# kursawe/OpticalFlow

Hardware: AMD Instinct MI355X
Metric: frame-pairs/sec (higher is better)
Workload: dtype f64; 1 GPU; 1024x1024x256 synthetic translating texture (seed 1), speed_alpha=1, remodelling_alpha=1e4, rtol=1e-06, all 255 pairs solved to the stopping rule; frames_per_gpu=256, pairs_in_flight=255, levels=9, coarse_stencils=float8, vcycle_vectors=coarse_float32, w_cycle_level=1, w_cycle_visits=3, warm_start_stride=3, allgather=False, gather_chunks=1, converged=True

## Files before the change

opticalflow_amd/csrc/vof.hip:

```cpp
#include "vof_device.hpp"
#include "vof_sweep0r.hpp"
#include "vof_sweep0p.hpp"
#include "vof_stream0.hpp"
#include "vof_direct.hpp"
#include "vof_boxflow.hpp"
#include "vof_boxsweep.hpp"
#include "vof_blursweep.hpp"
#include "vof_compare.hpp"
#include "vof_liushen.hpp"
#include "../../include/vof.h"

#include <fcntl.h>
#include <unistd.h>

#include <algorithm>
#include <atomic>
#include <chrono>
#include <cmath>
#include <condition_variable>
#include <cstdio>
#include <cstdlib>
#include <cstring>
#include <mutex>
#include <string>
// ... 49 lines not shown
    size_t warm_cap = 0;
    int* warm_src = nullptr;
    double* partials = nullptr;
    int nblk = 0;
    PairScalars* sc = nullptr;
    int* active = nullptr;
    int* alist = nullptr;
    int alist_n = 0;
    bool use_alist = true;
    double* func3 = nullptr;
    double *W = nullptr, *invT = nullptr;
    int nd = 0;
    int* h_active = nullptr;
    int* h_alist = nullptr;
    PairScalars* h_sc = nullptr;
    double* h_func3 = nullptr;
    char* h_bounce = nullptr;
    hipEvent_t ev_batch[2] = {nullptr, nullptr};
    double* st_movie = nullptr;
    double* st_out[4] = {nullptr, nullptr, nullptr, nullptr};
    double* st_out2[4] = {nullptr, nullptr, nullptr, nullptr};
    hipStream_t copy_stream = nullptr;
    hipEvent_t ev_solved[2] = {nullptr, nullptr}, ev_copied[2] = {nullptr, nullptr}, ev_uploaded[2] = {nullptr, nullptr};
    double* st_movie2 = nullptr;
    double *blur_tmp = nullptr, *blur_w = nullptr, *blur_io = nullptr;
    double* bf_scratch = nullptr;
    double* sw_scratch = nullptr;
    size_t sw_planes = 0;
    bool sw_by_budget = false;
    char* sw_aux = nullptr;
    size_t sw_aux_bytes = 0;
    bool bf_lds_set = false;
    bool bl_lds_set = false;
    bool ls_lds_set = false;
    double* tex_tab = nullptr;
    size_t tex_cap = 0;
    double* gm_V = nullptr;
    GmresState* gm_state = nullptr;
    double* gm_partials = nullptr;
    int* gm_cycle = nullptr;
    int gm_m = 0;
    long long gmres_pairs = 0;
    struct Alloc { void* raw; char* user; size_t bytes; const char* name; int line; };
    std::vector<Alloc> allocs;
    int c_bytes_per_point = 0;
    size_t bytes = 0;
    std::string err;
    const double* frames = nullptr;
    int npairs = 0;
    vof_params prm;
    int cfmt = 0;
    bool fused = true;
    bool fold_stored = false;
    bool direct_on = false;
    int dir_cap = 0;
    double *dir_T = nullptr, *dir_tabs = nullptr, *dir_W = nullptr, *dir_r = nullptr, *dir_y = nullptr, *dir_x = nullptr, *dir_t = nullptr;
    int *dir_ipiv = nullptr, *dir_info = nullptr;
    double *dir_R = nullptr, *dir_C = nullptr, *dir_D = nullptr;
    int dir_ld = 0;
    long long direct_pairs = 0;
    bool fuse_rr = true;
    bool fuse_b = true;
    int fused_ends = 3;
    long sweep0r_min_blocks = 512;
    int tail_first = -1;
    size_t tail_lds = 0;
    TailArgs tail;
    int tail_key[6] = {-9, -9, -9, -9, -9, -9};
    bool prof = false;
    int prof_kid = -1, prof_level = -1;
    std::vector<ProfRec> recs;
    std::vector<hipEvent_t> free_events;
    long long prof_dropped = 0;
    double prof_ms[VOF_K_COUNT][16];
    long long prof_n[VOF_K_COUNT][16];
    long long prof_units[VOF_K_COUNT][16];
    double prof_bytes[VOF_K_COUNT][16];
    double prof_moved[VOF_K_COUNT][16];
    int cur_units = 0;
    int dbg_sync = 0;
    long long dbg_seq = 0;
    std::string dbg_fault;
    int dbg_fd = -1;
    bool dbg_canary = false;
    bool dbg_alloc_log = false;
    bool dbg_poison = false;
    size_t part_per_pair = 0;
    vof_ctx* lane_parent = nullptr;
    int lane_lo = 0, lane_slots = 0;
    int dir_ok = -1;
    hipStream_t lane_stream[MAX_LANES] = {};
    hipEvent_t lane_ev[MAX_LANES][2] = {};
    hipEvent_t ev_fork = nullptr;
    hipEvent_t group_ev[MAX_LANES * MAX_LANE_GROUPS] = {};
};

static std::string g_create_error;

namespace {

void dbg_sync_check(vof_ctx* c, const char* what, int level) {
    if (!c->dbg_sync) return;
    ++c->dbg_seq;
    char line[256];
    if (c->dbg_fd >= 0) {
        int n = snprintf(line, sizeof line, "in flight: scope #%lld '%s' level %d, %d pairs, grid %dx%d (%d levels)%-40s\n", c->dbg_seq, what, level,
// ... 356 lines not shown
}

template <typename VT, typename CVT = VT>
void resrestrict_fine_t(vof_ctx* c, const VT* x, const VT* b, CVT* bc, int np, ActiveSet active) {
    Level &f = c->L[0], &k = c->L[1];
    int TI = pick_band_height(f.ni, (k.nj + RR_CO - 1) / RR_CO, c->cur_units);
    dim3 g((k.nj + RR_CO - 1) / RR_CO, (k.ni + TI / 2 - 1) / (TI / 2), pair_slots(c, active, np));
    Prof p(c, VOF_K_APPLY0, 0, (8.0 + 6.0 * sizeof(VT)) * f.npts + 3.0 * sizeof(CVT) * k.npts);
    k_stream_resrestrict0<VT, VT, CVT><<<g, AP_THREADS, 0, c->stream>>>(ap_args(c, TI, active), x, b, bc, k.ni, k.nj);
}

inline double resu_coef_bytes(const vof_ctx* c) {
    return c->cfmt == 3 ? 12.0 * 4 : (c->cfmt == 2 ? 18.5 * 4 : (c->cfmt == 1 ? 36.0 * 4 : 36.0 * 8));
}
template <typename VT>
void resrestrict_u_t(vof_ctx* c, int l, const VT* x_new, const VT* x_old, VT* bc, int np, ActiveSet active) {
    Level &f = c->L[l], &k = c->L[l + 1];
    const double vs = sizeof(VT);
    const double algo = (coef_bytes(c, l) + 9.0 * vs) * f.npts + 3.0 * vs * (f.npts + k.npts);
    const double moved = (resu_coef_bytes(c) + (x_old ? 6.0 : 3.0) * vs) * f.npts + 3.0 * vs * k.npts;
    Prof p(c, VOF_K_RESIDUAL, l, algo, moved);
    dim3 g(1, (k.ni + BY - 1) / BY, pair_slots(c, active, np));
    CDISPATCH(c, l, {
        if (x_old) k_resrestrict_u<CT, VT, true><<<g, blk2d, 0, c->stream>>>((const CW*)f.C, f.ni, f.nj, x_new, x_old, bc, k.ni, k.nj, active);
        else k_resrestrict_u<CT, VT, false><<<g, blk2d, 0, c->stream>>>((const CW*)f.C, f.ni, f.nj, x_new, x_old, bc, k.ni, k.nj, active);
    });
}

template <typename VT>
void prolong_add_level_t(vof_ctx* c, int l, VT* fine, const VT* coarse, int np, ActiveSet active) {
    Level &f = c->L[l], &k = c->L[l + 1];
    Prof p(c, VOF_K_PROLONG, l, 3.0 * sizeof(VT) * (2 * f.npts + k.npts));
    k_prolong_add<VT><<<grid2d(f.ni, f.nj, pair_slots(c, active, np)), blk2d, 0, c->stream>>>(fine, f.ni, f.nj, coarse, k.ni, k.nj, active);
}

template <typename VT>
void coarse_solve_t(vof_ctx* c, const VT* r, VT* e, int np, ActiveSet active) {
    Prof p(c, VOF_K_COARSE_SOLVE, (int)c->L.size() - 1);
    k_coarse_solve<VT><<<pair_slots(c, active, np), 256, c->nd * sizeof(double), c->stream>>>(c->invT, c->nd, r, e, active);
}

inline bool sweep0m_usable(const vof_ctx* c) {
    return c->fused && !c->vfloat && (c->L[0].nj % 2 == 0) && c->L[0].C == nullptr;
}

inline bool sweep0p_usable(const vof_ctx* c) {
    return c->fused && c->vfloat && (c->L[0].nj % 2 == 0) && c->L[0].C == nullptr && c->prm.reference_quirks;
}

inline bool sweep_st_usable(const vof_ctx* c, int l) {
    return l > 0 && c->L[l].C != nullptr && c->cfmt >= 2;
}

inline bool coarse32_ok(const vof_ctx* c, int nu_post) {
    return c->vcoarse32 && c->L.size() > 1 && sweep0m_usable(c) && nu_post > 0;
}


struct CycleIO {
    S0Trail trail{nullptr, nullptr, 0, nullptr};
    S0BSrc bf{nullptr, nullptr, nullptr, nullptr, nullptr, nullptr};
    int bf_mode = 0;
    int trail_nblk = 0;
    bool rr_done = false;
    bool bf_done = false;
    bool failed = false;
};

struct L0Req {
    bool from_zero = false;
    int po = 0;
    int nsweeps = 1;
    bool ec = false, ec32 = false;
    bool trail = false, trail_dot = false;
    bool rr = false, rr_f32 = false;
    int bf = 0;
    bool x32 = false;
};

enum L0Family { L0_SWEEP0R, L0_SWEEP0M, L0_SWEEP0P, L0_SWEEP0 };

struct L0Pass {
    L0Family fam = L0_SWEEP0;
    int NS = 1;
    bool EC = false, FROM_ZERO = false;
    int TRAIL = 0;
    bool ET32 = false;
    int PO = 0;
    int BF = 0;
    bool XT32 = false;
    int nx = 0, nxp = 0, ny = 0, TI = 0, nci = 0, ncj = 0;
    unsigned blocks = 0, block = 0;
    size_t lds = 0;
    double algo = 0.0, moved = 0.0;
    bool trail() const { return TRAIL == 1; }
    bool rr() const { return TRAIL == 2; }
    int bf() const { return BF == 3 ? 0 : BF; }
};

struct S0Geo { int nx, ny, TI; bool s0r; };
inline S0Geo s0_geometry(const vof_ctx* c, int rows, int NSW, bool trail) {
    const Level& lv = c->L[0];
    S0Geo g;
    const int out = S0_W - 8 * NSW - (trail ? 4 : 0);
    g.nx = (lv.nj + out - 1) / out;
    g.TI = pick_band_height(rows, g.nx, c->cur_units);
// ... 241 lines not shown
        {
            Prof pr(c, VOF_K_GS0, 0, p.algo, p.moved);
            const int nslots = pair_slots(c, active, np);
            switch (p.fam) {
                case L0_SWEEP0R: launched = launch_s0r(c, p, f0, nslots, ptrs); break;
                case L0_SWEEP0M: launched = launch_s0m(c, p, f0, nslots, ptrs); break;
                case L0_SWEEP0P: launched = launch_s0p(c, p, f0, nslots, ptrs); break;
                case L0_SWEEP0: launched = launch_s0<VT>(c, p, f0, nslots, ptrs); break;
            }
        }
        if (!launched) { c->err = "internal: the library holds no kernel for the planned level-0 pass"; io.failed = true; return; }
        if (p.trail()) io.trail_nblk = (int)p.blocks;
        if (p.rr()) io.rr_done = true;
        if (p.bf()) { io.bf_done = true; if (p.bf() == 1) fold_s_epilogue(c, np, p); }
        return;
    }
    const int rows = lv.ni + po;
    const int W = GeoB::W;
    const int nx = (lv.nj + GeoB::OUT - 1) / GeoB::OUT;
    const int TI = pick_band_height(rows, nx, c->cur_units);
    const int ny = (rows + TI - 1) / TI;
    const int nslots = pair_slots(c, active, np);
    dim3 g((unsigned)nx * ny * nslots, 1, 1);
    const double vs = sizeof(VT);
    int nci = 0, ncj = 0;
    double ebytes = 0.0;
    if (ecoarse) { nci = c->L[l + 1].ni; ncj = c->L[l + 1].nj; ebytes = 3.0 * vs * c->L[l + 1].npts; }
    Prof p(c, VOF_K_GS, l, (coef_bytes(c, l) + (x_in ? 9.0 : 6.0) * vs) * lv.npts + ebytes);
    size_t lds = (size_t)(SW_RING * 3 * W) * sizeof(VT);
    if (sweep_st_usable(c, l)) {
        const uint32_t* Cw = (const uint32_t*)lv.C;
        auto launch = [&](auto ct_tag) {
        using PCT = typename decltype(ct_tag)::type;
        if (ecoarse) {
            const size_t lds_e = lds + (size_t)9 * (W / 2 + 2) * sizeof(VT);
            if (a.out64) k_sweep_st<PCT, VT, double, true><<<g, GeoB::THREADS, lds_e, c->stream>>>(Cw, lv.ni, lv.nj, TI, po, nx, ny, nslots, x_in, (double*)x_out, b, active, ecoarse, nci, ncj, 0);
            else k_sweep_st<PCT, VT, VT, true><<<g, GeoB::THREADS, lds_e, c->stream>>>(Cw, lv.ni, lv.nj, TI, po, nx, ny, nslots, x_in, x_out, b, active, ecoarse, nci, ncj, 0);
        } else {
            const int sk = (a.skip0 && x_in && !a.reverse) ? 1 : 0;
            if (a.out64) k_sweep_st<PCT, VT, double><<<g, GeoB::THREADS, lds, c->stream>>>(Cw, lv.ni, lv.nj, TI, po, nx, ny, nslots, x_in, (double*)x_out, b, active, nullptr, 0, 0, sk);
            else k_sweep_st<PCT, VT><<<g, GeoB::THREADS, lds, c->stream>>>(Cw, lv.ni, lv.nj, TI, po, nx, ny, nslots, x_in, x_out, b, active, nullptr, 0, 0, sk);
        }
        };
        if (c->cfmt == 3) launch(TypeTag<CoefF8>{}); else launch(TypeTag<CoefB16>{});
        return;
    }
    CDISPATCH(c, l, {
        SweepStored<CT> pol; pol.C = (const CW*)lv.C; pol.plane = CLay(lv.ni, lv.nj).plane;
        k_sweep<SweepStored<CT>, GeoB, VT><<<g, GeoB::THREADS, lds, c->stream>>>(pol, lv.ni, lv.nj, TI, po, nx, ny, nslots, x_in, x_out, b, active, ecoarse, nci, ncj);
    });
}

template <typename VT>
VT* smooth_level_t(vof_ctx* c, int l, VT* x, VT* tmp, const VT* b, int nu, int np, ActiveSet active, SmoothArgs<VT> a, CycleIO& io) {
    const size_t bytes = (size_t)np * 3 * c->L[l].npts * sizeof(VT);
    const bool fine0 = l == 0 && c->L[0].C == nullptr;
    const bool fold = a.ecoarse && nu > 0 && c->fused && !a.from_zero && (fine0 || (sweep_st_usable(c, l) && c->fold_stored));
    if (a.ecoarse && !fold) {
        prolong_add_level_t<VT>(c, l, x, a.ecoarse, np, active);
        a.ecoarse = nullptr;
    }
    if (nu <= 0) {
        if (a.from_zero) hipMemsetAsync(x, 0, bytes, c->stream);
        return x;
    }
    if (!c->fused) {
        if (a.from_zero) hipMemsetAsync(x, 0, bytes, c->stream);
        for (int s = 0; s < nu; ++s)
            for (int k = 0; k < 4; ++k)
                gs_colour(c, l, (double*)x, (const double*)b, a.reverse ? 3 - k : k, np, active);
        return x;
    }
    L0Req two_rq;
    two_rq.nsweeps = 2;
    const bool two = fine0 && plan_l0_pass<VT>(c, two_rq).NS == 2;
    const int npass = two ? (nu + 1) / 2 : nu;
    const VT* src = a.from_zero ? nullptr : x;
    VT* dst = (a.from_zero && (npass % 2 == 1)) ? x : tmp;
    int left = nu;
    for (int s = 0; s < npass && !io.failed; ++s) {
        const bool first = s == 0, last = s == npass - 1;
        SmoothArgs<VT> pa = a;
        pa.nsweeps = two ? std::min(2, left) : 1;
        pa.trail = a.final_smooth && last && l == 0;
        if (!first) { pa.ecoarse = nullptr; pa.skip0 = false; }
        if (!last) { pa.out64 = false; pa.rr_out = nullptr; }
        sweep_level_t<VT>(c, l, src, dst, b, np, active, pa, io);
        left -= pa.nsweeps;
        src = dst;
        dst = (dst == x) ? tmp : x;
    }
    if (src != x) {
        if (a.allow_swap) return tmp;
        hipMemcpyAsync(x, src, bytes, hipMemcpyDeviceToDevice, c->stream);
    }
    return x;
}

void tail_emit(const vof_ctx* c, std::vector<unsigned char>* ops, int l, bool from_zero) {
    const vof_params& P = c->prm;
    const int last = (int)c->L.size() - 1, tl = l - c->tail_first;
    auto emit = [&](int code, int arg) { ops[0].push_back((unsigned char)code); ops[1].push_back((unsigned char)tl); ops[2].push_back((unsigned char)arg); };
    if (l == last) { emit(T_COARSE, 0); return; }
    const int nu1 = P.nu_pre_coarse > 0 ? P.nu_pre_coarse : P.nu_pre;
    const int nu2 = P.nu_post_coarse > 0 ? P.nu_post_coarse : P.nu_post;
    emit(T_SMOOTH, (nu1 << 2) | (from_zero ? 1 : 0));
    emit(T_RESTRICT, 0);
    tail_emit(c, ops, l + 1, true);
    if (P.w_cycle_level == l && l + 1 < last) {
        const int visits = P.w_cycle_visits > 0 ? P.w_cycle_visits : 2;
        for (int v = 1; v < visits; ++v) tail_emit(c, ops, l + 1, false);
    }
    emit(T_PROLONG, 0);
    emit(T_SMOOTH, (nu2 << 2) | 2);
}

bool tail_prepare(vof_ctx* c) {
    if (c->tail_first < 0 || !c->fused) return false;
    const vof_params& P = c->prm;
    const int key[6] = {P.nu_pre, P.nu_post, P.nu_pre_coarse, P.nu_post_coarse, P.w_cycle_level, P.w_cycle_visits};
    if (memcmp(key, c->tail_key, sizeof key) != 0) {
        std::vector<unsigned char> ops[3];
        tail_emit(c, ops, c->tail_first, true);
        memcpy(c->tail_key, key, sizeof key);
        if (ops[0].size() > (size_t)TAIL_MAX_OPS - 1 || std::max({P.nu_pre, P.nu_post, P.nu_pre_coarse, P.nu_post_coarse}) > 63) { c->tail.n_ops = -1; return false; }
        c->tail.n_ops = (int)ops[0].size();
        for (int i = 0; i < c->tail.n_ops; ++i) { c->tail.op[i] = ops[0][i]; c->tail.op_level[i] = ops[1][i]; c->tail.op_arg[i] = ops[2][i]; }
    }
    return c->tail.n_ops > 0;
}

template <typename VT>
void tail_cycle_t(vof_ctx* c, VT* x, const VT* b, int np, ActiveSet active, bool from_zero) {
    TailArgs A = c->tail;
    const int l0 = c->tail_first, last = (int)c->L.size() - 1;
    for (int l = l0; l <= last; ++l) A.L[l - l0].C = c->L[l].C;
    A.invT = c->invT;
    if (!from_zero) A.op_arg[0] &= ~1;
    const Level& top = c->L[l0];
    Prof p(c, VOF_K_COARSE_TAIL, l0, (from_zero ? 6.0 : 9.0) * sizeof(VT) * top.npts);
    CDISPATCH(c, l0, (k_tail_cycle<CT, VT><<<pair_slots(c, active, np), TAIL_THREADS, c->tail_lds, c->stream>>>(A, b, x, from_zero ? 1 : 0, active)));
}

template <typename VT>
VT* vcycle_t(vof_ctx* c, int l, VT* x, VT* tmp, const VT* b, int np, ActiveSet active, CycleIO& io, bool from_zero = true,
             bool after_post = false, bool emit64 = false) {
    int last = (int)c->L.size() - 1;
    if (l == last) { coarse_solve_t<VT>(c, b, x, np, active); return x; }
    if (l == c->tail_first && l > 0 && tail_prepare(c)) { tail_cycle_t<VT>(c, x, b, np, active, from_zero); return x; }
    Level& lv = c->L[l];
    Level& nx = c->L[l + 1];
    const int nu1 = (l > 0 && c->prm.nu_pre_coarse > 0) ? c->prm.nu_pre_coarse : c->prm.nu_pre;
    const int nu2 = (l > 0 && c->prm.nu_post_coarse > 0) ? c->prm.nu_post_coarse : c->prm.nu_post;
    const bool resu = l > 0 && lv.C != nullptr && c->fused && nu1 >= 1;
    SmoothArgs<VT> pre;
    pre.from_zero = from_zero;
    if (l == 0) {
        pre.rr_out = nx.b;
        pre.rr_f32 = coarse32_ok(c, nu2);
        io.rr_done = false;
    } else if (c->fused) {
        pre.allow_swap = true;
        pre.skip0 = after_post && !from_zero && nu2 >= 1;
    }
    if (smooth_level_t<VT>(c, l, x, tmp, b, nu1, np, active, pre, io) != x) std::swap(x, tmp);
    if (io.failed) return x;
    const bool rr_fused = l == 0 && io.rr_done;
    if constexpr (std::is_same<VT, double>::value) {
        if (l == 0 && coarse32_ok(c, nu2)) {
            if (!rr_fused) resrestrict_fine_t<double, float>(c, x, b, (float*)nx.b, np, active);
            float* fx = (float*)nx.x;
            float* ft = (float*)nx.x2;
            const int nu2c = c->prm.nu_post_coarse > 0 ? c->prm.nu_post_coarse : c->prm.nu_post;
            const bool can64 = 1 < last && !(c->tail_first == 1 && tail_prepare(c)) && sweep_st_usable(c, 1) && nu2c > 0;
            const int visits = (c->prm.w_cycle_level == 0 && 1 < last) ? (c->prm.w_cycle_visits > 0 ? c->prm.w_cycle_visits : 2) : 1;
            float* fe = vcycle_t<float>(c, 1, fx, ft, (const float*)nx.b, np, active, io, true, false, can64 && visits == 1);
            for (int v = 1; v < visits; ++v) {
                float* other = (fe == fx) ? ft : fx;
                fe = vcycle_t<float>(c, 1, fe, other, (const float*)nx.b, np, active, io, false, false, can64 && v == visits - 1);
            }
            SmoothArgs<double> post;
            post.reverse = post.allow_swap = post.final_smooth = true;
            post.ecoarse = (const double*)fe;
            post.ec32 = !can64;
            return smooth_level_t<double>(c, 0, x, tmp, b, nu2, np, active, post, io);
        }
    }
    if (resu) {
        const VT* x_old = (from_zero && nu1 == 1) ? nullptr : tmp;
        resrestrict_u_t<VT>(c, l, x, x_old, (VT*)nx.b, np, active);
    } else if (l == 0 && lv.C == nullptr) {
        if (!rr_fused) resrestrict_fine_t<VT>(c, x, b, (VT*)nx.b, np, active);
    } else {
        apply_level_t<VT>(c, l, x, b, (VT*)lv.r, 1, np, active);
        restrict_level_t<VT>(c, l, (const VT*)lv.r, (VT*)nx.b, np, active);
    }
    VT* cx = (VT*)nx.x;
    VT* ct = (VT*)nx.x2;
    VT* ec = vcycle_t<VT>(c, l + 1, cx, ct, (const VT*)nx.b, np, active, io, true);
    if (c->prm.w_cycle_level == l && l + 1 < last) {
        const int visits = c->prm.w_cycle_visits > 0 ? c->prm.w_cycle_visits : 2;
        for (int v = 1; v < visits; ++v) {
            VT* other = (ec == cx) ? ct : cx;
            ec = vcycle_t<VT>(c, l + 1, ec, other, (const VT*)nx.b, np, active, io, false, true);
        }
    }
    SmoothArgs<VT> post;
    post.reverse = post.allow_swap = true;
    post.final_smooth = l == 0;
    post.ecoarse = ec;
    post.out64 = emit64 && l == 1 && std::is_same<VT, float>::value && nu2 > 0;
    return smooth_level_t<VT>(c, l, x, tmp, b, nu2, np, active, post, io);
}

template <typename VT> int direct_apply_t(vof_ctx* c, VT* z, const VT* r, int np);

void vcycle(vof_ctx* c, double** xslot, const void* b, int np, ActiveSet active, CycleIO& io) {
    if (c->direct_on) {
        VDISPATCH(c, direct_apply_t<VT>(c, (VT*)*xslot, (const VT*)b, np));
        return;
    }
    void* res = nullptr;
    VDISPATCH(c, res = (void*)vcycle_t<VT>(c, 0, (VT*)*xslot, (VT*)c->L[0].x2, (const VT*)b, np, active, io));
    if (res != (void*)*xslot) {
        c->L[0].x2 = (void*)*xslot;
        *xslot = (double*)res;
    }
}

int build_hierarchy(vof_ctx* c, int np) {
    const vof_params& P = c->prm;
    c->cfmt = P.coarse_precision;
    int nl = (int)c->L.size();
    for (int l = 0; l + 1 < nl; ++l) {
        Level &f = c->L[l], &k = c->L[l + 1];
        dim3 g = grid2d(k.ni, k.nj, np);
        if (l == 0) {
            Prof p(c, VOF_K_GALERKIN0, 0);
            CDISPATCH(c, 1, (k_galerkin<double, CT, true><<<g, blk2d, 0, c->stream>>>(
                                 c->frames, frame_stride(c), c->Nj, P.speed_alpha, P.remodelling_alpha, P.reference_quirks,
                                 nullptr, f.ni, f.nj, (CW*)k.C, k.ni, k.nj, c->pp)));
        } else {
            Prof p(c, VOF_K_GALERKIN, l);
            CDISPATCH(c, 1, (k_galerkin<CT, CT, false><<<g, blk2d, 0, c->stream>>>(
                                 nullptr, 0, 0, 0.0, 0.0, 0, (const CW*)f.C, f.ni, f.nj, (CW*)k.C, k.ni, k.nj, nullptr)));
        }
    }
    return 0;
}

}

namespace vof {
__global__ __launch_bounds__(NT) void k_store_fine_stencil(const double* __restrict__ frames, size_t frame_stride,
                                                           int Nj, double alpha, double beta, int quirks, int ni,
                                                           int nj, double* __restrict__ C,
                                                           const PairParam* __restrict__ pp) {
    int q = blockIdx.x * BX + threadIdx.x, p = blockIdx.y * BY + threadIdx.y, pair = blockIdx.z;
    if (p >= ni || q >= nj) return;
    size_t npts = (size_t)ni * nj, idx = (size_t)p * nj + q;
    int fidx = pair;
    if (pp) { alpha = pp[pair].alpha; beta = pp[pair].beta; fidx = pp[pair].frame; }
    PixCoef k = pix_coef(frames + (size_t)fidx * frame_stride, Nj, p, q, quirks);
    const CLay L(ni, nj);
// ... 661 lines not shown
        std::string rep;
        if (dbg_check_canaries(c, &rep) != 0) { fprintf(stderr, "vof_destroy: VOF_DEBUG_CANARY: %s\n", rep.c_str()); fflush(stderr); }
    }
    if (c->dbg_fd >= 0) close(c->dbg_fd);
    prof_collect(c);
    for (auto e : c->free_events) hipEventDestroy(e);
    for (const auto& a : c->allocs) hipFree(a.raw);
    if (c->h_active) hipHostFree(c->h_active);
    if (c->h_alist) hipHostFree(c->h_alist);
    if (c->h_sc) hipHostFree(c->h_sc);
    if (c->h_func3) hipHostFree(c->h_func3);
    if (c->h_bounce) hipHostFree(c->h_bounce);
    for (int i = 0; i < 2; ++i) if (c->ev_batch[i]) hipEventDestroy(c->ev_batch[i]);
    for (int i = 0; i < 2; ++i) {
        if (c->ev_solved[i]) hipEventDestroy(c->ev_solved[i]);
        if (c->ev_copied[i]) hipEventDestroy(c->ev_copied[i]);
        if (c->ev_uploaded[i]) hipEventDestroy(c->ev_uploaded[i]);
    }
    if (c->copy_stream) hipStreamDestroy(c->copy_stream);
    for (int i = 0; i < MAX_LANES; ++i) {
        if (c->lane_stream[i]) hipStreamDestroy(c->lane_stream[i]);
        for (int j = 0; j < 2; ++j) if (c->lane_ev[i][j]) hipEventDestroy(c->lane_ev[i][j]);
    }
    if (c->ev_fork) hipEventDestroy(c->ev_fork);
    for (hipEvent_t e : c->group_ev) if (e) hipEventDestroy(e);
    if (c->own_stream && c->stream) hipStreamDestroy(c->stream);
    delete c;
}

static int create_impl(vof_ctx* c, int device_id, int n_i, int n_j, int B, void* stream) {
    if (n_i < 4 || n_j < 4) { c->err = "image must be at least 4x4 (the mirror boundary rows need N >= 4)"; return -1; }
    if (B < 1) { c->err = "max_pairs_in_flight must be >= 1"; return -1; }
    int ndev = 0;
    HIPCHK(hipGetDeviceCount(&ndev));
    if (device_id < 0 || device_id >= ndev) { c->err = "no such HIP device"; return -1; }
    HIPCHK(hipSetDevice(device_id));
    c->device = device_id;
    c->Ni = n_i; c->Nj = n_j; c->B = B;
    if (stream) { c->stream = (hipStream_t)stream; c->own_stream = false; }
    else { HIPCHK(hipStreamCreate(&c->stream)); c->own_stream = true; }
    memset(c->prof_ms, 0, sizeof c->prof_ms);
    memset(c->prof_n, 0, sizeof c->prof_n);
    memset(c->prof_units, 0, sizeof c->prof_units);
    memset(c->prof_bytes, 0, sizeof c->prof_bytes);
    memset(c->prof_moved, 0, sizeof c->prof_moved);
    vof_default_params(&c->prm, sizeof c->prm);
    if (const char* e = getenv("VOF_DEBUG_SYNC")) c->dbg_sync = atoi(e);
    if (const char* e = getenv("VOF_DEBUG_CANARY")) c->dbg_canary = e[0] != '0';
    if (const char* e = getenv("VOF_DEBUG_ALLOC_LOG")) c->dbg_alloc_log = e[0] != '0';
    if (const char* e = getenv("VOF_DEBUG_POISON")) c->dbg_poison = e[0] != '0';
    if (c->dbg_sync)
        if (const char* e = getenv("VOF_DEBUG_SYNC_FILE")) c->dbg_fd = open(e, O_WRONLY | O_CREAT, 0644);
    if (const char* e = getenv("VOF_FOLD_STORED")) c->fold_stored = e[0] != '0';
    if (const char* e = getenv("VOF_L0_HANDOFF")) c->l0_handoff = e[0] != '0';
    if (const char* e = getenv("VOF_SWEEP0R_MIN_BLOCKS")) c->sweep0r_min_blocks = atol(e);
    if (const char* e = getenv("VOF_ACTIVE_LIST")) c->use_alist = e[0] != '0';
    if (const char* e = getenv("VOF_FUSE_B")) c->fuse_b = e[0] != '0';
    if (const char* e = getenv("VOF_FUSE_RR")) c->fuse_rr = e[0] != '0';
    if (const char* e = getenv("VOF_FUSED_ENDS")) { const int v = atoi(e); if (v >= 0 && v <= 3) c->fused_ends = v; }
    Level l0; l0.ni = n_i - 2; l0.nj = n_j - 2; l0.npts = (size_t)l0.ni * l0.nj;
    c->L.push_back(l0);
    while (std::max(c->L.back().ni, c->L.back().nj) > COARSEST_MAX) {
        Level k; k.ni = (c->L.back().ni + 1) / 2; k.nj = (c->L.back().nj + 1) / 2; k.npts = (size_t)k.ni * k.nj;
        c->L.push_back(k);
    }
    int nl = (int)c->L.size();
    if (nl > 16) { c->err = "too many levels"; return -1; }
    size_t len0 = 3 * l0.npts;
    for (double** v : {&c->kx, &c->kb, &c->kr, &c->krh, &c->kp, &c->kv, &c->kt, &c->ky, &c->kz})
        if (int rc = dev_alloc(c, v, (size_t)B * len0)) return rc;
    for (int l = 0; l < nl; ++l) {
        Level& lv = c->L[l];
        auto valloc = [&](void** q) { double* t = nullptr; int rc = dev_alloc(c, &t, (size_t)B * 3 * lv.npts); *q = t; return rc; };
        if (l + 1 < nl && l > 0) if (int rc = valloc(&lv.r)) return rc;
        if (l + 1 < nl) if (int rc = valloc(&lv.x2)) return rc;
        if (l > 0) {
            if (int rc = valloc(&lv.x)) return rc;
            if (int rc = valloc(&lv.b)) return rc;
        }
        if (nl == 1) {
            double* C = nullptr;
            if (int rc = dev_alloc(c, &C, (size_t)B * 81 * CLay(lv.ni, lv.nj).plane)) return rc;
            lv.C = C;
        }
    }
    if (int rc = ensure_stencil_storage(c, vof_params_default_coarse_precision())) return rc;
    c->nd = 3 * (int)c->L.back().npts;
    {
        int first = -1;
        for (int l = 1; l < nl; ++l) {
            const CLay lay(c->L[l].ni, c->L[l].nj);
            if (c->L[l].npts <= (size_t)TAIL_MAX_PTS && lay.sub <= (size_t)TAIL_MAX_SUB) { first = l; break; }
        }
        if (first >= 0) first = std::max(first, nl - TAIL_MAX_LEVELS);
        if (first >= 1 && first < nl - 1) {
            memset(&c->tail, 0, sizeof c->tail);
            int off = 0;
            for (int l = first; l < nl; ++l) {
                TailLevel& t = c->tail.L[l - first];
                const CLay lay(c->L[l].ni, c->L[l].nj);
                t.ni = c->L[l].ni; t.nj = c->L[l].nj; t.hj = lay.hj; t.sub = (int)lay.sub; t.plane = lay.plane;
                t.xo = off; off += 3 * (t.ni + 2) * (t.nj + 2);
                t.bo = off; off += 3 * t.ni * t.nj;
            }
            c->tail.ro = off; off += 3 * (int)c->L[first].npts;
            c->tail.nl = nl - first;
            c->tail.nd = c->nd;
            c->tail.n_ops = 0;
            c->tail_lds = (size_t)off * sizeof(double);
            if (c->tail_lds <= (size_t)150 * 1024) {
                c->tail_first = first;
                const int lds = (int)c->tail_lds;
                HIPCHK(hipFuncSetAttribute((const void*)k_tail_cycle<CoefB16, double>, hipFuncAttributeMaxDynamicSharedMemorySize, lds));
                HIPCHK(hipFuncSetAttribute((const void*)k_tail_cycle<CoefB16, float>, hipFuncAttributeMaxDynamicSharedMemorySize, lds));
                HIPCHK(hipFuncSetAttribute((const void*)k_tail_cycle<CoefF8, double>, hipFuncAttributeMaxDynamicSharedMemorySize, lds));
                HIPCHK(hipFuncSetAttribute((const void*)k_tail_cycle<CoefF8, float>, hipFuncAttributeMaxDynamicSharedMemorySize, lds));
                HIPCHK(hipFuncSetAttribute((const void*)k_tail_cycle<float, double>, hipFuncAttributeMaxDynamicSharedMemorySize, lds));
                HIPCHK(hipFuncSetAttribute((const void*)k_tail_cycle<float, float>, hipFuncAttributeMaxDynamicSharedMemorySize, lds));
                HIPCHK(hipFuncSetAttribute((const void*)k_tail_cycle<double, double>, hipFuncAttributeMaxDynamicSharedMemorySize, lds));
                HIPCHK(hipFuncSetAttribute((const void*)k_tail_cycle<double, float>, hipFuncAttributeMaxDynamicSharedMemorySize, lds));
            }
        }
    }
    if (int rc = dev_alloc(c, &c->W, (size_t)B * c->nd * 2 * c->nd)) return rc;
    if (int rc = dev_alloc(c, &c->invT, (size_t)B * c->nd * c->nd)) return rc;
    {
        const int lds = 18 * s0_row_bytes(8) + 9 * (S0_W / 2 + 2) * 8;
        HIPCHK(hipFuncSetAttribute((const void*)k_sweep0m<2, true, false, 1>, hipFuncAttributeMaxDynamicSharedMemorySize, lds));
        HIPCHK(hipFuncSetAttribute((const void*)k_sweep0m<2, false, false, 1>, hipFuncAttributeMaxDynamicSharedMemorySize, lds));
        HIPCHK(hipFuncSetAttribute((const void*)k_sweep0m<1, true, false, 1>, hipFuncAttributeMaxDynamicSharedMemorySize, lds));
        HIPCHK(hipFuncSetAttribute((const void*)k_sweep0m<1, false, false, 1>, hipFuncAttributeMaxDynamicSharedMemorySize, lds));
    }
    c->nblk = (int)std::min<size_t>(256, std::max<size_t>(1, (len0 + 4 * RBLK - 1) / (4 * RBLK)));
    {
        int nblk_apply = ((l0.nj + AP_OUT - 1) / AP_OUT) * ((l0.ni + 31) / 32 + 1);
        nblk_apply = std::max(nblk_apply, ((l0.nj + 99) / 100) * ((l0.ni + 1 + 31) / 32 + 1));
        c->part_per_pair = (size_t)6 * std::max(c->nblk, nblk_apply);
        if (int rc = dev_alloc(c, &c->partials, (size_t)B * c->part_per_pair)) return rc;
    }
    if (int rc = dev_alloc(c, &c->sc, (size_t)B)) return rc;
    if (int rc = dev_alloc(c, &c->active, (size_t)B)) return rc;
    if (int rc = dev_alloc(c, &c->alist, (size_t)B)) return rc;
    if (int rc = dev_alloc(c, &c->func3, (size_t)B * 3)) return rc;
    HIPCHK(hipHostMalloc((void**)&c->h_active, B * sizeof(int)));
    HIPCHK(hipHostMalloc((void**)&c->h_alist, B * sizeof(int)));
    HIPCHK(hipHostMalloc((void**)&c->h_sc, B * sizeof(PairScalars)));
    HIPCHK(hipHostMalloc((void**)&c->h_func3, B * 3 * sizeof(double)));
    for (int i = 0; i < 2; ++i) HIPCHK(hipEventCreate(&c->ev_batch[i]));
    return 0;
}

int vof_create(vof_ctx** out, int device_id, int n_i, int n_j, int max_pairs_in_flight, void* stream) {
    if (!out) { g_create_error = "out is NULL"; return -1; }
    *out = nullptr;
    vof_ctx* c = new (std::nothrow) vof_ctx();
    if (!c) { g_create_error = "out of host memory"; return -1; }
    int rc = create_impl(c, device_id, n_i, n_j, max_pairs_in_flight, stream);
    if (rc) {
        g_create_error = c->err;
        vof_destroy(c);
        return rc;
    }
    *out = c;
    return 0;
}

}

namespace {

double lanes_min_pixels() {
    double mpix = 16.0;
    if (const char* e = getenv("VOF_LANES_MIN_MPIX")) { const double v = atof(e); if (v >= 0.0) mpix = v; }
    return mpix * 1e6;
}

int lanes_for(const vof_ctx* c, int pairs_per_phase) {
    if (c->prof || c->dbg_sync) return 1;
    int n = 3;
    if (const char* e = getenv("VOF_LANES")) { const int v = atoi(e); if (v >= 1 && v <= MAX_LANES) n = v; }
    const double minpix = lanes_min_pixels();
    n = std::min(n, c->B);
    while (n > 1 && (pairs_per_phase < n || (double)pairs_per_phase / n * c->Ni * c->Nj < minpix)) --n;
    return n;
// ... 2010 lines not shown
```

opticalflow_amd/csrc/vof_device.hpp:

```cpp
#pragma once
#include <hip/hip_runtime.h>
#include <stdint.h>
#include <type_traits>

namespace vof {

constexpr int BX = 64;
constexpr int BY = 4;
constexpr int NT = BX * BY;

struct PairScalars {
    double rho, alpha, omega, beta;
    double bnorm2, rnorm2;
    double tol2;
    int iterations;
    int converged;
    int breakdown;
    int halfstep;
};

struct PairParam {
    double alpha, beta;
    int frame;
    int out;
// ... 2059 lines not shown
                    for (int f = 0; f < 3; ++f) {
                        double v = wi0 * wj0 * (double)c0[f * CRW];
                        if (ipj) v += wi0 * 0.5 * (double)c0[f * CRW + 1];
                        if (ipi) {
                            v += 0.5 * wj0 * (double)c1[f * CRW];
                            if (ipj) v += 0.25 * (double)c1[f * CRW + 1];
                        }
                        lx[f] = (VT)((double)lx[f] + v);
                    }
                }
            }
            VT* lrow = xs + (m5.row ? slotB : slotA) * 3 * W + m5.lds;
            lrow[0] = lx[0]; lrow[W] = lx[1]; lrow[2 * W] = lx[2];
        }
        if (EC && do_load) {
            const CMap cm = cmap(opaque_tid());
            if (cm.on) cr[(cr_slot(knew) * 3 + cm.f) * CRW + cm.c] = (cm.cv && kok) ? crv : (VT)0;
        }
        slotA = sw_wrap(slotA + 2);
        __syncthreads();
    };

    const int s_end = TI / 2 + 4;
    const int e_lo = max(10, 10 - p0);
    const int e_hi = min(TI - 2, ni - 4 - p0);
    auto pair_fast = [&](const int s) { return 2 * s >= e_lo && 2 * (s + 1) <= e_hi; };
    auto run = [&](auto mask_tag) {
        int s = -2;
        for (int part = 0; part < 2; ++part) {
            while (s <= s_end && (part == 1 || !pair_fast(s))) {
                step(std::false_type{}, std::integral_constant<int, 0>{}, mask_tag, 2 * s);
                if (s + 1 <= s_end) step(std::false_type{}, std::integral_constant<int, 1>{}, mask_tag, 2 * (s + 1));
                s += 2;
            }
            if (part == 0 && s <= s_end) {
                __builtin_amdgcn_s_waitcnt(0x0F70);
                while (pair_fast(s)) {
                    step(std::true_type{}, std::integral_constant<int, 0>{}, mask_tag, 2 * s);
                    step(std::true_type{}, std::integral_constant<int, 1>{}, mask_tag, 2 * (s + 1));
                    s += 2;
                }
            }
        }
    };
    if (skip0 && po == 0 && wave == 0) {
        run(std::integral_constant<unsigned, SWST_NO_UPDATE>{});
    } else if (!x_in && po == 0 && wave < 4) {
        if (wave == 0) run(std::integral_constant<unsigned, 0x000u>{});
        else if (wave == 1) run(std::integral_constant<unsigned, 0x028u>{});
        else if (wave == 2) run(std::integral_constant<unsigned, 0x1C7u>{});
        else run(std::integral_constant<unsigned, 0x1EFu>{});
    } else {
        run(std::integral_constant<unsigned, 0x1EFu>{});
    }
}

struct Fine0 {
    const double* frames;
    size_t frame_stride;
    int Nj;
    double alpha, beta;
    int quirks;
    const PairParam* pp;
};
constexpr int S0_W = 128, S0_IW = 132, S0_OUT = 120, S0_THREADS = 256;
__host__ __device__ constexpr int s0_row_bytes(int vt_bytes) { return 3 * S0_W * vt_bytes + S0_IW * 8; }

template <typename VT, bool EC, bool FROM_ZERO>
__global__ __launch_bounds__(S0_THREADS) void k_sweep0(Fine0 pol, int ni, int nj, int TI, int po, int nx, int ny, int nz,
                                                       const VT* __restrict__ x_in, VT* __restrict__ x_out,
                                                       const VT* __restrict__ b, const ActiveSet act,
                                                       const VT* __restrict__ ecoarse, int nci, int ncj) {
    constexpr int W = S0_W, IW = S0_IW, OUT = S0_OUT;
    constexpr int VB = (int)sizeof(VT);
    constexpr int FB = W * VB;
    constexpr int XB = 3 * FB;
    constexpr int RSB = s0_row_bytes(VB);
    constexpr int RINGB = SW_RING * RSB;
    constexpr int CRW = W / 2 + 2;
    extern __shared__ double sw_lds[];
    char* ring = reinterpret_cast<char*>(sw_lds);
    VT* cr = reinterpret_cast<VT*>(ring + RINGB);
    const unsigned nblocks = (unsigned)nx * ny * nz;
    unsigned lb = blockIdx.x;
    if ((nblocks & 7u) == 0) lb = (lb & 7u) * (nblocks >> 3) + (lb >> 3);
    const int bx = lb % nx, by = (lb / nx) % ny;
    const int pair = act.pair(lb / (nx * ny));
    if (!act.on(pair)) return;
    const int tid = threadIdx.x, lane = tid & 63;
    const int wave = __builtin_amdgcn_readfirstlane(tid >> 6);
    const int p0 = by * TI - po;
    const int qs = bx * OUT - po - SW_HALO;
    const size_t npts = (size_t)ni * nj, off = (size_t)pair * 3 * npts;
    const VT* xin = FROM_ZERO ? nullptr : x_in + off;
    VT* xout = x_out + off;
    const VT* bp = b + off;
    const size_t ncpts = (size_t)nci * ncj;
    const VT* ec = EC ? ecoarse + (size_t)pair * 3 * ncpts : nullptr;
    double alpha = pol.alpha, beta = pol.beta;
    int fidx = pair;
    if (pol.pp) { alpha = pol.pp[pair].alpha; beta = pol.pp[pair].beta; fidx = pol.pp[pair].frame; }
    const double* img = pol.frames + (size_t)fidx * pol.frame_stride;
    const int Nj = pol.Nj, quirks = pol.quirks;
    const double inv_g = 1.0 / (-1 - 4 * beta);

    auto cs = [](int lc) { return (lc & 1) * (W / 2) + (lc >> 1); };
// ... 919 lines not shown
```

Before: 1423 frame-pairs/s.

## Fuse W-cycle revisit post-smooth and next pre-smooth into one two-sweep kernel

During W-cycle revisits at coarse stored-stencil levels, the post-smooth of one visit is deferred and merged with the pre-smooth of the next visit. A new k_sweep_st2 kernel runs the reverse and forward Gauss-Seidel sweeps in a single launch using a deeper LDS ring, and it writes both the intermediate and the final iterate. This removes one launch and one global reread of the iterate per revisit. In exchange the kernel carries more LDS and register pressure, needs a third buffer, and depends on extra wave-staging logic. A profiling script for comparing the launches is also added.

```diff
diff --git a/opticalflow_amd/csrc/vof.hip b/opticalflow_amd/csrc/vof.hip
--- a/opticalflow_amd/csrc/vof.hip
+++ b/opticalflow_amd/csrc/vof.hip
@@ -125,6 +125,7 @@
     int cfmt = 0;
     bool fused = true;
     bool fold_stored = false;
+    bool fuse_revisit = true;
     bool direct_on = false;
     int dir_cap = 0;
     double *dir_T = nullptr, *dir_tabs = nullptr, *dir_W = nullptr, *dir_r = nullptr, *dir_y = nullptr, *dir_x = nullptr, *dir_t = nullptr;
@@ -587,6 +588,15 @@
     return l > 0 && c->L[l].C != nullptr && c->cfmt >= 2;
 }
 
+bool tail_prepare(vof_ctx* c);
+inline bool revisit_fusable(vof_ctx* c, int l) {
+    if (!c->fused || !c->fuse_revisit || c->fold_stored || !sweep_st_usable(c, l) || l >= (int)c->L.size() - 1) return false;
+    if (l == c->tail_first && tail_prepare(c)) return false;
+    const int nu1 = c->prm.nu_pre_coarse > 0 ? c->prm.nu_pre_coarse : c->prm.nu_pre;
+    const int nu2 = c->prm.nu_post_coarse > 0 ? c->prm.nu_post_coarse : c->prm.nu_post;
+    return nu1 == 1 && nu2 == 1;
+}
+
 inline bool coarse32_ok(const vof_ctx* c, int nu_post) {
     return c->vcoarse32 && c->L.size() > 1 && sweep0m_usable(c) && nu_post > 0;
 }
@@ -934,6 +944,22 @@
 }
 
 template <typename VT>
+void sweep2_level_t(vof_ctx* c, int l, const VT* x_in, VT* x_mid, VT* x_out, const VT* b, int np, ActiveSet active) {
+    Level& lv = c->L[l];
+    const int nx = (lv.nj + GeoR::OUT - 1) / GeoR::OUT;
+    const int TI = pick_band_height(lv.ni, nx, c->cur_units);
+    const int ny = (lv.ni + TI - 1) / TI;
+    const int nslots = pair_slots(c, active, np);
+    dim3 g((unsigned)nx * ny * nslots, 1, 1);
+    const double vs = sizeof(VT);
+    Prof p(c, VOF_K_GS, l, 2.0 * (coef_bytes(c, l) + 9.0 * vs) * lv.npts, (coef_bytes(c, l) + 12.0 * vs) * lv.npts);
+    const size_t lds = (size_t)(GeoR::RING * 3 * GeoR::W) * sizeof(VT);
+    const uint32_t* Cw = (const uint32_t*)lv.C;
+    if (c->cfmt == 3) k_sweep_st2<CoefF8, VT><<<g, GeoR::THREADS, lds, c->stream>>>(Cw, lv.ni, lv.nj, TI, nx, ny, nslots, x_in, x_mid, x_out, b, active);
+    else k_sweep_st2<CoefB16, VT><<<g, GeoR::THREADS, lds, c->stream>>>(Cw, lv.ni, lv.nj, TI, nx, ny, nslots, x_in, x_mid, x_out, b, active);
+}
+
+template <typename VT>
 VT* smooth_level_t(vof_ctx* c, int l, VT* x, VT* tmp, const VT* b, int nu, int np, ActiveSet active, SmoothArgs<VT> a, CycleIO& io) {
     const size_t bytes = (size_t)np * 3 * c->L[l].npts * sizeof(VT);
     const bool fine0 = l == 0 && c->L[0].C == nullptr;
@@ -1026,7 +1052,7 @@
 
 template <typename VT>
 VT* vcycle_t(vof_ctx* c, int l, VT* x, VT* tmp, const VT* b, int np, ActiveSet active, CycleIO& io, bool from_zero = true,
-             bool after_post = false, bool emit64 = false) {
+             bool after_post = false, bool emit64 = false, bool defer_post = false, bool post_pending = false) {
     int last = (int)c->L.size() - 1;
     if (l == last) { coarse_solve_t<VT>(c, b, x, np, active); return x; }
     if (l == c->tail_first && l > 0 && tail_prepare(c)) { tail_cycle_t<VT>(c, x, b, np, active, from_zero); return x; }
@@ -1045,7 +1071,13 @@
         pre.allow_swap = true;
         pre.skip0 = after_post && !from_zero && nu2 >= 1;
     }
-    if (smooth_level_t<VT>(c, l, x, tmp, b, nu1, np, active, pre, io) != x) std::swap(x, tmp);
+    if (post_pending) {
+        VT* third = (VT*)lv.x;
+        if (third == x || third == tmp) third = (VT*)lv.x2;
+        if (third == x || third == tmp) third = (VT*)lv.r;
+        sweep2_level_t<VT>(c, l, x, tmp, third, b, np, active);
+        x = third;
+    } else if (smooth_level_t<VT>(c, l, x, tmp, b, nu1, np, active, pre, io) != x) std::swap(x, tmp);
     if (io.failed) return x;
     const bool rr_fused = l == 0 && io.rr_done;
     if constexpr (std::is_same<VT, double>::value) {
@@ -1056,10 +1088,12 @@
             const int nu2c = c->prm.nu_post_coarse > 0 ? c->prm.nu_post_coarse : c->prm.nu_post;
             const bool can64 = 1 < last && !(c->tail_first == 1 && tail_prepare(c)) && sweep_st_usable(c, 1) && nu2c > 0;
             const int visits = (c->prm.w_cycle_level == 0 && 1 < last) ? (c->prm.w_cycle_visits > 0 ? c->prm.w_cycle_visits : 2) : 1;
-            float* fe = vcycle_t<float>(c, 1, fx, ft, (const float*)nx.b, np, active, io, true, false, can64 && visits == 1);
+            const bool fr = visits > 1 && revisit_fusable(c, 1);
+            float* fe = vcycle_t<float>(c, 1, fx, ft, (const float*)nx.b, np, active, io, true, false, can64 && visits == 1, fr);
             for (int v = 1; v < visits; ++v) {
                 float* other = (fe == fx) ? ft : fx;
-                fe = vcycle_t<float>(c, 1, fe, other, (const float*)nx.b, np, active, io, false, false, can64 && v == visits - 1);
+                fe = vcycle_t<float>(c, 1, fe, other, (const float*)nx.b, np, active, io, false, false, can64 && v == visits - 1,
+                                     fr && v < visits - 1, fr);
             }
             SmoothArgs<double> post;
             post.reverse = post.allow_swap = post.final_smooth = true;
@@ -1079,19 +1113,23 @@
     }
     VT* cx = (VT*)nx.x;
     VT* ct = (VT*)nx.x2;
-    VT* ec = vcycle_t<VT>(c, l + 1, cx, ct, (const VT*)nx.b, np, active, io, true);
-    if (c->prm.w_cycle_level == l && l + 1 < last) {
-        const int visits = c->prm.w_cycle_visits > 0 ? c->prm.w_cycle_visits : 2;
-        for (int v = 1; v < visits; ++v) {
-            VT* other = (ec == cx) ? ct : cx;
-            ec = vcycle_t<VT>(c, l + 1, ec, other, (const VT*)nx.b, np, active, io, false, true);
-        }
+    const int visits = (c->prm.w_cycle_level == l && l + 1 < last) ? (c->prm.w_cycle_visits > 0 ? c->prm.w_cycle_visits : 2) : 1;
+    const bool fr = visits > 1 && revisit_fusable(c, l + 1);
+    VT* ec = vcycle_t<VT>(c, l + 1, cx, ct, (const VT*)nx.b, np, active, io, true, false, false, fr);
+    for (int v = 1; v < visits; ++v) {
+        VT* other = (ec == cx) ? ct : cx;
+        ec = vcycle_t<VT>(c, l + 1, ec, other, (const VT*)nx.b, np, active, io, false, true, false,
+                          fr && v < visits - 1, fr);
     }
     SmoothArgs<VT> post;
     post.reverse = post.allow_swap = true;
     post.final_smooth = l == 0;
     post.ecoarse = ec;
     post.out64 = emit64 && l == 1 && std::is_same<VT, float>::value && nu2 > 0;
+    if (defer_post) {
+        prolong_add_level_t<VT>(c, l, x, ec, np, active);
+        return x;
+    }
     return smooth_level_t<VT>(c, l, x, tmp, b, nu2, np, active, post, io);
 }
 
@@ -1859,6 +1897,7 @@
     if (c->dbg_sync)
         if (const char* e = getenv("VOF_DEBUG_SYNC_FILE")) c->dbg_fd = open(e, O_WRONLY | O_CREAT, 0644);
     if (const char* e = getenv("VOF_FOLD_STORED")) c->fold_stored = e[0] != '0';
+    if (const char* e = getenv("VOF_FUSE_REVISIT")) c->fuse_revisit = e[0] != '0';
     if (const char* e = getenv("VOF_L0_HANDOFF")) c->l0_handoff = e[0] != '0';
     if (const char* e = getenv("VOF_SWEEP0R_MIN_BLOCKS")) c->sweep0r_min_blocks = atol(e);
     if (const char* e = getenv("VOF_ACTIVE_LIST")) c->use_alist = e[0] != '0';
@@ -1937,6 +1976,11 @@
         HIPCHK(hipFuncSetAttribute((const void*)k_sweep0m<2, false, false, 1>, hipFuncAttributeMaxDynamicSharedMemorySize, lds));
         HIPCHK(hipFuncSetAttribute((const void*)k_sweep0m<1, true, false, 1>, hipFuncAttributeMaxDynamicSharedMemorySize, lds));
         HIPCHK(hipFuncSetAttribute((const void*)k_sweep0m<1, false, false, 1>, hipFuncAttributeMaxDynamicSharedMemorySize, lds));
+    }
+    {
+        const int lds = GeoR::RING * 3 * GeoR::W * (int)sizeof(double);
+        HIPCHK(hipFuncSetAttribute((const void*)k_sweep_st2<CoefB16, double>, hipFuncAttributeMaxDynamicSharedMemorySize, lds));
+        HIPCHK(hipFuncSetAttribute((const void*)k_sweep_st2<CoefF8, double>, hipFuncAttributeMaxDynamicSharedMemorySize, lds));
     }
     c->nblk = (int)std::min<size_t>(256, std::max<size_t>(1, (len0 + 4 * RBLK - 1) / (4 * RBLK)));
     {
diff --git a/opticalflow_amd/csrc/vof_device.hpp b/opticalflow_amd/csrc/vof_device.hpp
--- a/opticalflow_amd/csrc/vof_device.hpp
+++ b/opticalflow_amd/csrc/vof_device.hpp
@@ -2135,6 +2135,245 @@
         else run(std::integral_constant<unsigned, 0x1EFu>{});
     } else {
         run(std::integral_constant<unsigned, 0x1EFu>{});
+    }
+}
+
+struct GeoR {
+    static constexpr int OUT = 128, HALO = 8, W = 144, THREADS = 512, RING = 22;
+};
+template <typename CT, typename VT>
+__global__ __launch_bounds__(GeoR::THREADS, SweepStBudget<CT>::kMinWaves) void k_sweep_st2(const typename CoefFmt<CT>::word_t* __restrict__ C, int ni, int nj, int TI,
+                                                               int nx, int ny, int nz, const VT* __restrict__ x_in,
+                                                               VT* __restrict__ x_mid, VT* __restrict__ x_out,
+                                                               const VT* __restrict__ b, const ActiveSet act) {
+    typedef GeoR G;
+    typedef typename CoefFmt<CT>::word_t word_t;
+    constexpr int W = G::W, OUT = G::OUT, HALO = G::HALO, RING = G::RING, PLANES = CoefFmt<CT>::PLANES;
+    extern __shared__ double sw_lds[];
+    VT* xs = reinterpret_cast<VT*>(sw_lds);
+    const unsigned nblocks = (unsigned)nx * ny * nz;
+    unsigned lb = blockIdx.x;
+    if ((nblocks & 7u) == 0) lb = (lb & 7u) * (nblocks >> 3) + (lb >> 3);
+    const int bx = lb % nx, by = (lb / nx) % ny;
+    const int pair = act.pair(lb / (nx * ny));
+    if (!act.on(pair)) return;
+    const int tid = threadIdx.x, lane = tid & 63;
+    const int wave = __builtin_amdgcn_readfirstlane(tid >> 6);
+    const int H = TI + 4;
+    const int p0 = by * TI - 1;
+    const int qs = bx * OUT - HALO;
+    const size_t npts = (size_t)ni * nj, off = (size_t)pair * 3 * npts;
+    const VT* xin = x_in + off;
+    VT* xmid = x_mid + off;
+    VT* xout = x_out + off;
+    const VT* bp = b + off;
+    const CLay L(ni, nj);
+    const word_t* Cp = C + (size_t)pair * PLANES * L.plane;
+
+    int stage = wave, lc;
+    bool lane_on = true;
+    lc = HALO + 2 * lane + ((wave & 1) ^ 1);
+    if (wave == 7) {
+        constexpr int NH = 21;
+        const int hs[NH] = {0, 0, 0, 0, 0, 0, 1, 1, 1, 1, 1, 2, 2, 2, 2, 3, 3, 3, 4, 4, 5};
+        const int hl[NH] = {3, 5, 7, HALO + OUT + 1, HALO + OUT + 3, HALO + OUT + 5, 4, 6, HALO + OUT, HALO + OUT + 2, HALO + OUT + 4,
+                            5, 7, HALO + OUT + 1, HALO + OUT + 3, 6, HALO + OUT, HALO + OUT + 2, 7, HALO + OUT + 1, HALO + OUT};
+        lane_on = lane < NH;
+        stage = hs[lane_on ? lane : 0];
+        lc = hl[lane_on ? lane : 0];
+    }
+    const int q = qs + lc;
+    const bool col_ok = lane_on && (q >= 0) && (q < nj);
+    const int qc = col_ok ? q : 0, lcc = col_ok ? lc : 2;
+    const int cC = sw_cs<G>(lcc), uL = sw_cs<G>(lcc - 1), uR = sw_cs<G>(lcc + 1);
+    const unsigned ccq = (unsigned)((size_t)(qc & 1) * L.sub + (size_t)(qc >> 1));
+    const unsigned bcol = (unsigned)qc;
+    auto opaque_tid = [&]() { int t = tid; asm volatile("" : "+v"(t)); return t; };
+    struct XMap { int row, col, q, lds; unsigned g; bool on, ld, st; };
+    auto xmap = [&](const int t) {
+        XMap m;
+        m.row = t >= W ? 1 : 0; m.col = t - m.row * W;
+        m.on = t < 2 * W;
+        m.q = qs + m.col;
+        m.ld = m.on && m.q >= 0 && m.q < nj;
+        m.st = m.ld && m.col >= HALO && m.col < HALO + OUT;
+        m.g = m.ld ? (unsigned)m.q : 0u;
+        m.lds = sw_cs<G>(m.on ? m.col : 0);
+        return m;
+    };
+    auto wrap = [](int t) { return t >= RING ? t - RING : t; };
+    const int sro = (stage == 0) ? 0 : (stage == 1) ? -2 : (stage == 2) ? -5 : (stage == 3) ? -7 : (stage == 4) ? -11 : (stage == 5) ? -14 : -16;
+    const int rr_lo = (stage < 2) ? 0 : (stage < 5) ? 1 : 2;
+    const int rr_hi = (stage < 2) ? H : (stage < 4) ? H - 1 : (stage == 4) ? TI + 1 : TI;
+    const bool uni = wave < 7;
+
+    constexpr int ND = CoefFmt<CT>::ND;
+    constexpr bool F8 = std::is_same<CT, CoefF8>::value;
+    static_assert(CoefPacked<CT>::value, "k_sweep_st2 is written for the packed stencil formats");
+    word_t cw[2][ND], dg[PLANES - ND];
+    VT bq[3];
+#pragma unroll
+    for (int k = 0; k < ND; ++k) cw[0][k] = cw[1][k] = 0;
+#pragma unroll
+    for (int k = 0; k < PLANES - ND; ++k) dg[k] = 0;
+    bq[0] = bq[1] = bq[2] = (VT)0;
+    auto offd = [](const word_t* w, int j) {
+        if constexpr (F8) {
+            return (double)f8_decode(w[j >> 2], j & 3);
+        } else {
+            const uint32_t v = w[j >> 1];
+            return (double)__uint_as_float((j & 1) ? (v & 0xFFFF0000u) : (v << 16));
+        }
+    };
+    auto point_base = [&](const int pn, const word_t*& base, unsigned& idx, const bool fast) {
+        if (fast && uni) {
+            const int pnu = __builtin_amdgcn_readfirstlane(pn);
+            base = Cp + (size_t)((pnu & 1) << 1) * L.sub + (size_t)(pnu >> 1) * L.hj;
+            idx = ccq;
+        } else {
+            base = Cp;
+            idx = (unsigned)((size_t)((pn & 1) << 1) * L.sub + (size_t)(pn >> 1) * L.hj) + ccq;
+        }
+    };
+    auto fetch_point = [&](auto fast_tag, auto jtag, const int eN) {
+        constexpr bool FAST = decltype(fast_tag)::value;
+        constexpr int J = decltype(jtag)::value;
+        const int rrn = eN + sro, pn = p0 + rrn;
+        if (FAST || (col_ok && rrn >= rr_lo && rrn <= rr_hi && pn >= 0 && pn < ni)) {
+            const word_t* base; unsigned idx;
+            point_base(pn, base, idx, FAST);
+#pragma unroll
+            for (int k = 0; k < ND; ++k) cw[J][k] = (base + (size_t)k * L.plane)[idx];
+        }
+    };
+    auto fetch_diag = [&](auto fast_tag, const int eN) {
+        constexpr bool FAST = decltype(fast_tag)::value;
+        const int rrn = eN + sro, pn = p0 + rrn;
+        if (FAST || (col_ok && rrn >= rr_lo && rrn <= rr_hi && pn >= 0 && pn < ni)) {
+            const word_t* base; unsigned idx;
+            point_base(pn, base, idx, FAST);
+#pragma unroll
+            for (int k = 0; k < PLANES - ND; ++k) dg[k] = (base + (size_t)(ND + k) * L.plane)[idx];
+            const VT* brow = bp + (size_t)pn * nj + bcol;
+            bq[0] = brow[0]; bq[1] = brow[npts]; bq[2] = brow[2 * npts];
+        }
+    };
+
+    int slotA = (2 * RING - 2) % RING;
+    auto step = [&](auto fast_tag, auto jtag, const int e) {
+        constexpr bool FAST = decltype(fast_tag)::value;
+        constexpr int JC = decltype(jtag)::value;
+        const bool do_load = FAST ? true : (e + 2 <= H + 1);
+        const XMap m1 = xmap(opaque_tid());
+        {
+            const int rr = e - 10 + m1.row, p = p0 + rr;
+            if (m1.st && (FAST || (rr >= 1 && rr <= TI && p >= 0 && p < ni))) {
+                VT* orow = xmid + (size_t)p * nj + m1.g;
+                const VT* lrow = xs + (wrap(slotA + RING - 12) + m1.row) * 3 * W + m1.lds;
+                orow[0] = lrow[0]; orow[npts] = lrow[W]; orow[2 * npts] = lrow[2 * W];
+            }
+        }
+        {
+            const int rr = e - 20 + m1.row, p = p0 + rr;
+            if (m1.st && (FAST || (rr >= 1 && rr <= TI && p >= 0 && p < ni))) {
+                VT* orow = xout + (size_t)p * nj + m1.g;
+                const VT* lrow = xs + (slotA + m1.row) * 3 * W + m1.lds;
+                orow[0] = lrow[0]; orow[npts] = lrow[W]; orow[2 * npts] = lrow[2 * W];
+            }
+        }
+        VT lx[3] = {(VT)0, (VT)0, (VT)0};
+        {
+            const int pR = p0 + e + 2 + m1.row;
+            if (FAST) {
+                const VT* irow = xin + (size_t)pR * nj + m1.g;
+                lx[0] = irow[0]; lx[1] = irow[npts]; lx[2] = irow[2 * npts];
+            } else if (m1.ld && do_load && pR >= 0 && pR < ni) {
+                const VT* irow = xin + (size_t)pR * nj + m1.g;
+                lx[0] = irow[0]; lx[1] = irow[npts]; lx[2] = irow[2 * npts];
+            }
+        }
+        fetch_point(fast_tag, std::integral_constant<int, 1 - JC>{}, e + 2);
+        {
+            const int rr = e + sro, p = p0 + rr;
+            if (col_ok && (FAST || (rr >= rr_lo && rr <= rr_hi && p >= 0 && p < ni))) {
+                const int sU = wrap(slotA + RING + sro - 3), sC = wrap(slotA + RING + sro - 2), sD = wrap(slotA + RING + sro - 1);
+                const int rowo[3] = {sU * 3 * W, sC * 3 * W, sD * 3 * W};
+                const int colo[3] = {uL, cC, uR};
+                const word_t* c_ = cw[JC];
+                double y0 = 0, y1 = 0, y2 = 0;
+                typedef double AT;
+                AT yp[F8 ? 9 : 1];
+                if constexpr (F8) {
+#pragma unroll
+                    for (int t = 0; t < 9; ++t) yp[t] = 0;
+                }
+#pragma unroll
+                for (int a = 0; a < 3; ++a) {
+                    const VT* row = xs + rowo[a];
+#pragma unroll
+                    for (int bb = 0; bb < 3; ++bb) {
+                        if (a == 1 && bb == 1) continue;
+                        double xu = (double)row[colo[bb]], xw = (double)row[W + colo[bb]], xg = (double)row[2 * W + colo[bb]];
+                        const int d = a * 3 + bb, t0 = (d < 4 ? d : d - 1) * 9;
+                        if constexpr (F8) {
+                            const AT au = (AT)row[colo[bb]], aw = (AT)row[W + colo[bb]], ag = (AT)row[2 * W + colo[bb]];
+#pragma unroll
+                            for (int r = 0; r < 3; ++r) {
+                                yp[3 * r + 0] += (AT)f8_decode(c_[(t0 + 3 * r + 0) >> 2], (t0 + 3 * r + 0) & 3) * au;
+                                yp[3 * r + 1] += (AT)f8_decode(c_[(t0 + 3 * r + 1) >> 2], (t0 + 3 * r + 1) & 3) * aw;
+                                yp[3 * r + 2] += (AT)f8_decode(c_[(t0 + 3 * r + 2) >> 2], (t0 + 3 * r + 2) & 3) * ag;
+                            }
+                        } else {
+                            y0 += offd(c_, t0 + 0) * xu + offd(c_, t0 + 1) * xw + offd(c_, t0 + 2) * xg;
+                            y1 += offd(c_, t0 + 3) * xu + offd(c_, t0 + 4) * xw + offd(c_, t0 + 5) * xg;
+                            y2 += offd(c_, t0 + 6) * xu + offd(c_, t0 + 7) * xw + offd(c_, t0 + 8) * xg;
+                        }
+                    }
+                    asm volatile("" ::: "memory");
+                }
+                double Dm[9];
+#pragma unroll
+                for (int t = 0; t < 9; ++t) Dm[t] = (double)__uint_as_float(dg[t]);
+                if constexpr (F8) {
+                    y0 = (double)yp[0] * (double)f8_unit(dg[9], 0) + (double)yp[1] * (double)f8_unit(dg[9], 1) + (double)yp[2] * (double)f8_unit(dg[9], 2);
+                    y1 = (double)yp[3] * (double)f8_unit(dg[10], 0) + (double)yp[4] * (double)f8_unit(dg[10], 1) + (double)yp[5] * (double)f8_unit(dg[10], 2);
+                    y2 = (double)yp[6] * (double)f8_unit(dg[11], 0) + (double)yp[7] * (double)f8_unit(dg[11], 1) + (double)yp[8] * (double)f8_unit(dg[11], 2);
+                }
+                double u, w, gm;
+                solve3(Dm, (double)bq[0] - y0, (double)bq[1] - y1, (double)bq[2] - y2, u, w, gm);
+                VT* row = xs + rowo[1] + cC;
+                row[0] = (VT)u; row[W] = (VT)w; row[2 * W] = (VT)gm;
+            }
+        }
+        fetch_diag(fast_tag, e + 2);
+        const XMap m5 = xmap(opaque_tid());
+        if (do_load && m5.on) {
+            VT* lrow = xs + (slotA + m5.row) * 3 * W + m5.lds;
+            lrow[0] = lx[0]; lrow[W] = lx[1]; lrow[2 * W] = lx[2];
+        }
+        slotA = wrap(slotA + 2);
+        __syncthreads();
+    };
+
+    const int s_end = TI / 2 + 10;
+    const int e_lo = max(22, 20 - p0);
+    const int e_hi = min(TI + 2, ni - 4 - p0);
+    auto pair_fast = [&](const int s) { return 2 * s >= e_lo && 2 * (s + 1) <= e_hi; };
+    int s = -2;
+    for (int part = 0; part < 2; ++part) {
+        while (s <= s_end && (part == 1 || !pair_fast(s))) {
+            step(std::false_type{}, std::integral_constant<int, 0>{}, 2 * s);
+            if (s + 1 <= s_end) step(std::false_type{}, std::integral_constant<int, 1>{}, 2 * (s + 1));
+            s += 2;
+        }
+        if (part == 0 && s <= s_end) {
+            __builtin_amdgcn_s_waitcnt(0x0F70);
+            while (pair_fast(s)) {
+                step(std::true_type{}, std::integral_constant<int, 0>{}, 2 * s);
+                step(std::true_type{}, std::integral_constant<int, 1>{}, 2 * (s + 1));
+                s += 2;
+            }
+        }
     }
 }
 
diff --git a/profiles/revisit_launches.py b/profiles/revisit_launches.py
--- /dev/null
+++ b/profiles/revisit_launches.py
@@ -0,0 +1,64 @@
+#!/usr/bin/env python3
+import csv
+import re
+import sys
+from collections import defaultdict
+from statistics import median
+
+
+def short(name):
+    return re.sub(r"\(.*", "", name).replace("void ", "").replace("vof::", "").strip()
+
+
+def rows_of(mode, path):
+    per_queue = defaultdict(list)
+    with open(path) as f:
+        for r in csv.DictReader(f):
+            if mode == "trace":
+                grid = int(r["Grid_Size_X"]) * int(r.get("Grid_Size_Y", 1) or 1) * int(r.get("Grid_Size_Z", 1) or 1)
+                t0, t1 = int(r["Start_Timestamp"]), int(r["End_Timestamp"])
+                per_queue[r.get("Queue_Id", "?")].append((t0, short(r["Kernel_Name"]), grid, (t1 - t0) / 1e3))
+            else:
+                per_queue[r.get("Queue_Id", "?")].append((int(r["Dispatch_Id"]), short(r["Kernel_Name"]), int(r["Grid_Size"]),
+                                                         float(r["Counter_Value"])))
+    for q in per_queue.values():
+        q.sort()
+    return per_queue
+
+
+def main():
+    mode, path = sys.argv[1], sys.argv[2]
+    per_queue = rows_of(mode, path)
+    total = sum(v for q in per_queue.values() for _, _, _, v in q)
+    single = defaultdict(list)
+    pairs = defaultdict(list)
+    fused = defaultdict(list)
+    for q in per_queue.values():
+        i = 0
+        while i < len(q):
+            _, name, grid, v = q[i]
+            if name.startswith("k_sweep_st2<"):
+                fused[grid].append(v)
+            elif name.startswith("k_sweep_st<"):
+                single[(name, grid)].append(v)
+                if i + 1 < len(q) and q[i + 1][1].startswith("k_sweep_st<"):
+                    single[(q[i + 1][1], q[i + 1][2])].append(q[i + 1][3])
+                    pairs[(grid, q[i + 1][2])].append((v, q[i + 1][3]))
+                    i += 1
+            i += 1
+    unit = "us" if mode == "trace" else "counter"
+    print(f"all kernels: {total:.1f} {unit}")
+    print(f"\n| k_sweep_st launches | grid (threads) | launches | total | median |\n|---|---:|---:|---:|---:|")
+    for (name, grid), v in sorted(single.items(), key=lambda kv: -sum(kv[1])):
+        print(f"| `{name}` | {grid} | {len(v)} | {sum(v):.1f} | {median(v):.1f} |")
+    print(f"\n| back-to-back pairs: grids | pairs | total | median first | median second | median of the sum |\n|---|---:|---:|---:|---:|---:|")
+    for (ga, gb), v in sorted(pairs.items(), key=lambda kv: -sum(a + b for a, b in kv[1])):
+        print(f"| {ga} + {gb} | {len(v)} | {sum(a + b for a, b in v):.1f} | {median(a for a, _ in v):.1f} | {median(b for _, b in v):.1f} | "
+              f"{median(a + b for a, b in v):.1f} |")
+    print(f"\n| k_sweep_st2: grid | launches | total | median |\n|---|---:|---:|---:|")
+    for grid, v in sorted(fused.items(), key=lambda kv: -sum(kv[1])):
+        print(f"| {grid} | {len(v)} | {sum(v):.1f} | {median(v):.1f} |")
+
+
+if __name__ == "__main__":
+    main()
```

After: 1446 frame-pairs/s, median of 6. 1.6% higher.
